# Intelligent-Driving-Laboratory/GOPS

Hardware: NVIDIA H100
Metric: batched env-steps/sec (FHADP rollout+update) (higher is better)
Workload: dtype f32

## Files before the change

### gops_b200/csrc/rollout_tc2.cuh

```cuda
#pragma once
#include "models.cuh"
#include "mlp_tc_full.cuh"
#include "tc2_probe.cuh"

namespace gops {
namespace tc2 {

constexpr int WGS = 3;
constexpr int GT = 64;
constexpr int NT2 = 128 * WGS;
constexpr int HPL = tcf::HPLANE, XPL = tcf::XPLANE;
constexpr int P_BYTES = 3 * HPL, Q_BYTES = 2 * HPL, XP_BYTES = 3 * XPL;
constexpr int GROUP_BYTES = P_BYTES + Q_BYTES + 2 * XP_BYTES;
constexpr int HDR_BYTES = 256;

__host__ __device__ inline size_t smem_bytes(int w_floats) {
  return HDR_BYTES + (size_t)w_floats * 4 + tcf::ONES_B + (size_t)WGS * GROUP_BYTES;
}

__device__ __forceinline__ void split2(f32x2::u64 X, uint32_t& p0, uint32_t& p1) {
  float r0, r1;
  f32x2::upk(X, r0, r1);
  asm("cvt.rn.bf16x2.f32 %0, %1, %2;" : "=r"(p0) : "f"(r1), "f"(r0));
  f32x2::upk(f32x2::fma(tcf::bf16x2_as_f32x2(p0), f32x2::rep(-1.f), X), r0, r1);
  asm("cvt.rn.bf16x2.f32 %0, %1, %2;" : "=r"(p1) : "f"(r1), "f"(r0));
}

__device__ __forceinline__ void red_add(float* p, float v) {
  asm volatile("red.global.add.f32 [%0], %1;" ::"l"(p), "f"(v) : "memory");
}
__device__ __forceinline__ void red_add2(float* p, float v0, float v1) {
  asm volatile("red.global.add.v2.f32 [%0], {%1, %2};" ::"l"(p), "f"(v0), "f"(v1) : "memory");
}

struct Grp {
  unsigned char* P;
  const float* Wsm;
  int g, t, c;
  int row;
  bool own;
  __device__ __forceinline__ unsigned char* Q() const { return P + P_BYTES; }
  __device__ __forceinline__ unsigned char* X(int k) const { return P + P_BYTES + Q_BYTES + (k & 1) * XP_BYTES; }
  __device__ __forceinline__ const unsigned char* ones() const {
    return reinterpret_cast<const unsigned char*>(Wsm) - tcf::ONES_B;
  }
  __device__ __forceinline__ const unsigned char* W1(const NetL& L) const { return reinterpret_cast<const unsigned char*>(Wsm + L.o_w1); }
  __device__ __forceinline__ const unsigned char* W2(const NetL& L) const { return reinterpret_cast<const unsigned char*>(Wsm + L.o_w2); }
  __device__ __forceinline__ const float* W3(const NetL& L) const { return Wsm + L.o_w3; }
  __device__ __forceinline__ const float* b1(const NetL& L) const { return Wsm + L.o_b1; }
  __device__ __forceinline__ const float* b2(const NetL& L) const { return Wsm + L.o_b2; }
  __device__ __forceinline__ const float* b3(const NetL& L) const { return Wsm + L.o_b3; }
};

__device__ __forceinline__ void publish(const Grp& G) {
  fence_proxy_async();
  wg::wg_sync(G.g);
}

template <int N, int TB, int KS>
__device__ __forceinline__ void mma6(float* d, const tcf::Op& A, const tcf::Op& B) {
  using namespace tcf;
  const uint64_t a0 = dsc(A, 0), a1 = dsc(A, 1), a2 = dsc(A, 2), b0 = dsc(B, 0), b1 = dsc(B, 1), b2 = dsc(B, 2);
  const uint64_t ka = A.kadv >> 4, kb = B.kadv >> 4;
#pragma unroll
  for (int ks = 0; ks < KS; ++ks) wg::mma_bf16<N, 0, TB>(d, a2 + ks * ka, b0 + ks * kb, ks > 0 ? 1u : 0u);
#pragma unroll
  for (int ks = 0; ks < KS; ++ks) wg::mma_bf16<N, 0, TB>(d, a0 + ks * ka, b2 + ks * kb, 1u);
#pragma unroll
  for (int ks = 0; ks < KS; ++ks) wg::mma_bf16<N, 0, TB>(d, a1 + ks * ka, b1 + ks * kb, 1u);
#pragma unroll
  for (int ks = 0; ks < KS; ++ks) wg::mma_bf16<N, 0, TB>(d, a1 + ks * ka, b0 + ks * kb, 1u);
#pragma unroll
  for (int ks = 0; ks < KS; ++ks) wg::mma_bf16<N, 0, TB>(d, a0 + ks * ka, b1 + ks * kb, 1u);
#pragma unroll
  for (int ks = 0; ks < KS; ++ks) wg::mma_bf16<N, 0, TB>(d, a0 + ks * ka, b0 + ks * kb, 1u);
}
template <int N, int KS>
__device__ __forceinline__ void mma_dw(float* d, const tcf::Op& A, const tcf::Op& B) {
  using namespace tcf;
  const uint64_t a0 = dsc(A, 0), a1 = dsc(A, 1), b0 = dsc(B, 0), b1 = dsc(B, 1);
  const uint64_t ka = A.kadv >> 4, kb = B.kadv >> 4;
#pragma unroll
  for (int ks = 0; ks < KS; ++ks) wg::mma_bf16<N, 0, 1>(d, a1 + ks * ka, b0 + ks * kb, ks > 0 ? 1u : 0u);
#pragma unroll
  for (int ks = 0; ks < KS; ++ks) wg::mma_bf16<N, 0, 1>(d, a0 + ks * ka, b1 + ks * kb, 1u);
#pragma unroll
  for (int ks = 0; ks < KS; ++ks) wg::mma_bf16<N, 0, 1>(d, a0 + ks * ka, b0 + ks * kb, 1u);
}
template <int N, int BP>
__device__ __forceinline__ void mma_wgrad(float* d, const tcf::Op& A, const tcf::Op& B) {
  using namespace tcf;
  const uint64_t ka = A.kadv >> 4, kb = B.kadv >> 4;
  uint32_t acc = 0u;
#pragma unroll
  for (int p = BP - 1; p >= 0; --p)
#pragma unroll
    for (int q = 1; q >= 0; --q) {
      const uint64_t a = dsc(A, q), b = dsc(B, p);
#pragma unroll
      for (int ks = 0; ks < GT / 16; ++ks) { wg::mma_bf16<N, 1, 1>(d, a + ks * ka, b + ks * kb, acc); acc = 1u; }
    }
}
__device__ __forceinline__ tcf::Op ones_op(const Grp& G) { return tcf::Op{smem_u32(G.ones()), 0u, 128u, 256u, 0u}; }

template <int NP>
__device__ __forceinline__ void frag_to_planes(unsigned char* buf, const Grp& G, const float* v) {
#pragma unroll
  for (int i = 0; i < 32; i += 2) {
    const int off = (i >> 2) * (GT * 16) + wg::frag_row(G.t, i) * 16 + 4 * G.c;
    uint32_t w0, w1, w2;
    if constexpr (NP == 3) tcf::split3(v[i], v[i + 1], w0, w1, w2);
    else split2(f32x2::pk(v[i], v[i + 1]), w0, w1);
    *reinterpret_cast<uint32_t*>(buf + off) = w0;
    *reinterpret_cast<uint32_t*>(buf + HPL + off) = w1;
    if constexpr (NP == 3) *reinterpret_cast<uint32_t*>(buf + 2 * HPL + off) = w2;
  }
}
template <int N, bool PAIRS>
__device__ __forceinline__ void red_frag(float* __restrict__ dst, int ld, int ncols, const float* d, int t) {
#pragma unroll
  for (int i = 0; i < N / 2; i += 2) {
    const int row = wg::frag_row(t, i), col = wg::frag_col(t, i);
    if constexpr (PAIRS) {
      red_add2(dst + row * ld + col, d[i], d[i + 1]);
    } else {
      if (col < ncols) red_add(dst + row * ld + col, d[i]);
      if (col + 1 < ncols) red_add(dst + row * ld + col + 1, d[i + 1]);
    }
  }
}
__device__ __forceinline__ void red_bias(float* __restrict__ dst, const float* d, const Grp& G) {
  if (G.c == 0) {
    red_add(dst + wg::frag_row(G.t, 0), d[0]);
    red_add(dst + wg::frag_row(G.t, 2), d[2]);
  }
}

template <int NS>
__device__ __forceinline__ void put_x(const Grp& G, unsigned char* x, const NetL& L, const float* st, float vt) {
  using namespace tcf;
  if (!G.own) return;
  float v[16];
#pragma unroll
  for (int f = 0; f < 16; ++f) v[f] = (f < NS && f < L.obs) ? st[f < NS ? f : 0] : 0.f;
  if (L.time_input) {
#pragma unroll
    for (int f = 0; f < 16; ++f)
      if (f == L.in - 1) v[f] = vt;
  }
  const int nch = L.in <= 8 ? 1 : 2;
#pragma unroll
  for (int ch = 0; ch < 2; ++ch) {
    if (ch >= nch) break;
    uint32_t w[3][4];
#pragma unroll
    for (int i = 0; i < 4; ++i) split3(v[8 * ch + 2 * i], v[8 * ch + 2 * i + 1], w[0][i], w[1][i], w[2][i]);
#pragma unroll
    for (int p = 0; p < 3; ++p)
      *reinterpret_cast<uint4*>(x + p * XPL + (ch * GT + G.row) * 16) = make_uint4(w[p][0], w[p][1], w[p][2], w[p][3]);
  }
}

#define GOPS_TC2_ACT_SWITCH(AF, act, M)     \
  if constexpr ((AF) >= 0) { M(AF); }       \
  else { GOPS_ACT_SWITCH(act, M) }

__device__ __forceinline__ void layer1_issue(const Grp& G, const NetL& L, const unsigned char* x, float* d) {
  using namespace tcf;
  publish(G);
  wg::fence();
  mma6<64, 0, 1>(d, k_act(x, XPL), k_w(G.W1(L), W1PLANE));
  wg::commit();
}
template <bool FULL, int AF>
__device__ __forceinline__ void layer1_finish(const Grp& G, const NetL& L, float* d, float* a1p) {
  wg::wait<0>();
  wg::reg_fence<32>(d);
#define GOPS_TC2_A1(A)                                                                             \
  _Pragma("unroll") for (int i = 0; i < 32; i += 2) {                                              \
    const f32x2::u64 pre = f32x2::add(f32x2::pk(d[i], d[i + 1]), f32x2::ld(G.b1(L) + wg::frag_col(G.t, i))); \
    if constexpr (FULL) act_fwd_grad_pair_t<A>(pre, d[i], d[i + 1], a1p[i], a1p[i + 1]);           \
    else act_fwd_pair_t<A>(pre, d[i], d[i + 1]);                                                   \
  }
  GOPS_TC2_ACT_SWITCH(AF, L.hact, GOPS_TC2_A1)
#undef GOPS_TC2_A1
  frag_to_planes<3>(G.P, G, d);
}

__device__ __forceinline__ void layer2_product(const Grp& G, const NetL& L, float* d) {
  using namespace tcf;
  publish(G);
  wg::fence();
  mma6<64, 0, 4>(d, k_act(G.P, HPL), k_w(G.W2(L), W2PLANE));
  wg::commit();
  wg::wait<0>();
  wg::reg_fence<32>(d);
}
template <int NA>
__device__ __forceinline__ bool live(int a, const NetL& L) { return NA == 1 || a < L.out; }

template <int NA>
__device__ __forceinline__ void output_sum(const Grp& G, const NetL& L, f32x2::u64 (*S)[NA], float* z) {
#pragma unroll
  for (int a = 0; a < NA; ++a) {
    z[a] = 0.f;
    if (live<NA>(a, L)) {
      float s[2];
#pragma unroll
      for (int q = 0; q < 2; ++q) {
        float s0, s1;
        f32x2::upk(S[q][a], s0, s1);
        s[q] = s0 + s1;
        s[q] += __shfl_xor_sync(0xffffffffu, s[q], 1);
        s[q] += __shfl_xor_sync(0xffffffffu, s[q], 2);
      }
      z[a] = G.b3(L)[a] + (G.c == 0 ? s[0] : s[1]);
    }
  }
}
template <int NA>
__device__ __forceinline__ void output_layer(const Grp& G, const NetL& L, const float* h, float* z) {
  f32x2::u64 S[2][NA];
#pragma unroll
  for (int a = 0; a < NA; ++a) S[0][a] = S[1][a] = f32x2::rep(0.f);
#pragma unroll
  for (int i = 0; i < 32; i += 2) {
    const int col = wg::frag_col(G.t, i), q = (i >> 1) & 1;
#pragma unroll
    for (int a = 0; a < NA; ++a)
      if (live<NA>(a, L)) S[q][a] = f32x2::fma(f32x2::ld(G.W3(L) + a * 64 + col), f32x2::pk(h[i], h[i + 1]), S[q][a]);
  }
  output_sum<NA>(G, L, S, z);
}

template <int AF, int NA>
__device__ __forceinline__ void layer2_out(const Grp& G, const NetL& L, float* z) {
  float d[32];
  layer2_product(G, L, d);
#define GOPS_TC2_A2(A)                                \
  _Pragma("unroll") for (int i = 0; i < 32; i += 2)   \
      act_fwd_pair_t<A>(f32x2::add(f32x2::pk(d[i], d[i + 1]), f32x2::ld(G.b2(L) + wg::frag_col(G.t, i))), d[i], d[i + 1]);
  GOPS_TC2_ACT_SWITCH(AF, L.hact, GOPS_TC2_A2)
#undef GOPS_TC2_A2
  output_layer<NA>(G, L, d, z);
}

template <int NA>
struct Acc3 {
  float w[NA][2];
  float b[NA];
};

template <int A, bool WANT_DW, bool WANT_Z, int NA>
__device__ __forceinline__ void delta2_epilogue(const Grp& G, const NetL& L, float* d, const float (*zr)[NA],
                                                Acc3<NA>& acc3, f32x2::u64 (*S)[NA]) {
  const int q4 = (G.t & 31) >> 2;
#pragma unroll
  for (int j = 0; j < 8; ++j) {
    const int col = 8 * j + 2 * G.c;
    float h[2][2];
#pragma unroll
    for (int q = 0; q < 2; ++q) {
      const int i = 4 * j + 2 * q;
      float g0, g1;
      act_fwd_grad_pair_t<A>(f32x2::add(f32x2::pk(d[i], d[i + 1]), f32x2::ld(G.b2(L) + col)), h[q][0], h[q][1], g0, g1);
      f32x2::u64 gs = f32x2::rep(0.f);
#pragma unroll
      for (int a = 0; a < NA; ++a)
        if (live<NA>(a, L)) gs = f32x2::fma(f32x2::ld(G.W3(L) + a * 64 + col), f32x2::rep(zr[q][a]), gs);
      uint32_t w0, w1;
      split2(f32x2::mul(f32x2::pk(g0, g1), gs), w0, w1);
      const int off = j * (GT * 16) + wg::frag_row(G.t, i) * 16 + 4 * G.c;
      *reinterpret_cast<uint32_t*>(G.Q() + off) = w0;
      *reinterpret_cast<uint32_t*>(G.Q() + HPL + off) = w1;
      if constexpr (WANT_Z) {
#pragma unroll
        for (int a = 0; a < NA; ++a)
          if (live<NA>(a, L)) S[q][a] = f32x2::fma(f32x2::ld(G.W3(L) + a * 64 + col), f32x2::pk(h[q][0], h[q][1]), S[q][a]);
      }
    }
    if constexpr (WANT_DW) {
#pragma unroll
      for (int a = 0; a < NA; ++a)
        if (live<NA>(a, L)) {
#pragma unroll
          for (int e = 0; e < 2; ++e) {
            float v = fmaf(zr[1][a], h[1][e], zr[0][a] * h[0][e]);
            v += __shfl_xor_sync(0xffffffffu, v, 4);
            v += __shfl_xor_sync(0xffffffffu, v, 8);
            v += __shfl_xor_sync(0xffffffffu, v, 16);
            if (q4 == j) acc3.w[a][e] += v;
          }
        }
    }
  }
}

template <bool WANT_DW, bool WANT_Z, int AF, int NA>
__device__ __forceinline__ void layer2_back(const Grp& G, const NetL& L, const float* zbar, float* z, Acc3<NA>& acc3) {
  float d[32];
  layer2_product(G, L, d);
  const int qb = (G.t & 31) & ~3;
  float zr[2][NA];
#pragma unroll
  for (int a = 0; a < NA; ++a) {
    zr[0][a] = __shfl_sync(0xffffffffu, zbar[a], qb);
    zr[1][a] = __shfl_sync(0xffffffffu, zbar[a], qb + 1);
  }
  f32x2::u64 S[2][NA];
#pragma unroll
  for (int a = 0; a < NA; ++a) S[0][a] = S[1][a] = f32x2::rep(0.f);
#define GOPS_TC2_A3(A) delta2_epilogue<A, WANT_DW, WANT_Z, NA>(G, L, d, zr, acc3, S);
  GOPS_TC2_ACT_SWITCH(AF, L.hact, GOPS_TC2_A3)
#undef GOPS_TC2_A3
  if constexpr (WANT_Z) output_sum<NA>(G, L, S, z);
  if constexpr (WANT_DW) {
#pragma unroll
    for (int a = 0; a < NA; ++a)
      if (live<NA>(a, L) && G.own) acc3.b[a] += zbar[a];
  }
}

template <bool WANT_DW, int NS, bool OVERLAP>
__device__ __forceinline__ void backprop(const Grp& G, const NetL& L, bool want_dx, float* __restrict__ part,
                                         const unsigned char* x, const float* a1p, float* dx, Probe& pr) {
  using namespace tcf;
  publish(G);
  constexpr bool overlap = WANT_DW && OVERLAP;
  float g1[32], w[32], wb[8];
  wg::fence();
  mma_dw<64, 4>(g1, k_act(G.Q(), HPL), mn_w(G.W2(L), W2PLANE));
  wg::commit();
  if constexpr (overlap) {
    mma_wgrad<64, 2>(w, mn_act(G.Q(), HPL), mn_act(G.P, HPL));
    mma_wgrad<16, 1>(wb, mn_act(G.Q(), HPL), ones_op(G));
    wg::commit();
    wg::wait<1>();
  } else {
    wg::wait<0>();
  }
  wg::reg_fence<32>(g1);
  if (!WANT_DW && !want_dx) return;
#pragma unroll
  for (int i = 0; i < 32; ++i) g1[i] *= a1p[i];
  if constexpr (WANT_DW) {
    if constexpr (!overlap) {
      wg::fence();
      mma_wgrad<64, 2>(w, mn_act(G.Q(), HPL), mn_act(G.P, HPL));
      mma_wgrad<16, 1>(wb, mn_act(G.Q(), HPL), ones_op(G));
      wg::commit();
    }
    wg::wait<0>();
    wg::reg_fence<32>(w);
    wg::reg_fence<8>(wb);
    red_frag<64, true>(part + L.g_w2, 64, 64, w, G.t);
    red_bias(part + L.g_b2, wb, G);
  }
  pr.stamp(kRevD2);
  wg::wg_sync(G.g);
  frag_to_planes<2>(G.Q(), G, g1);
  publish(G);
  float d[8], w1[8], wb1[8];
  if (want_dx) {
    wg::fence();
    mma_dw<16, 4>(d, k_act(G.Q(), HPL), mn_w(G.W1(L), W1PLANE));
    wg::commit();
  }
  if constexpr (WANT_DW) {
    wg::fence();
    mma_wgrad<16, 2>(w1, mn_act(G.Q(), HPL), mn_act(x, XPL));
    mma_wgrad<16, 1>(wb1, mn_act(G.Q(), HPL), ones_op(G));
    wg::commit();
  }
  wg::wait<0>();
  if constexpr (WANT_DW) {
    wg::reg_fence<8>(w1);
    wg::reg_fence<8>(wb1);
    red_frag<16, false>(part + L.g_w1, L.in, L.in, w1, G.t);
    red_bias(part + L.g_b1, wb1, G);
  }
  if (want_dx) {
    wg::reg_fence<8>(d);
    const int qb = (G.t & 31) & ~3;
#pragma unroll
    for (int j = 0; j < 2; ++j)
#pragma unroll
      for (int cc = 0; cc < 4; ++cc)
#pragma unroll
        for (int e = 0; e < 2; ++e) {
          const int f = 8 * j + 2 * cc + e;
          if (f < NS) {
            const float v0 = __shfl_sync(0xffffffffu, d[4 * j + e], qb + cc);
            const float v1 = __shfl_sync(0xffffffffu, d[4 * j + 2 + e], qb + cc);
            dx[f] = G.c == 0 ? v0 : v1;
          }
        }
  }
}

}

template <class M, int ALG, int AF, int NA, class W>
__global__ void __launch_bounds__(tc2::NT2, 1) rollout_tc2_kernel(const __grid_constant__ KParams p) {
  using namespace tc2;
  static_assert(M::KIND == 0, "wgmma rollout kernel: state == obs models");
  static_assert(NA == 1 || NA == MAXA, "wgmma rollout kernel: NA is MAXA or 1");
  constexpr int NS = M::NS, alg = ALG;
  extern __shared__ __align__(16) float smem[];
  unsigned char* sm = reinterpret_cast<unsigned char*>(smem);
  uint64_t* bars = reinterpret_cast<uint64_t*>(sm);
  unsigned char* ones = sm + HDR_BYTES;
  float* Wsm = reinterpret_cast<float*>(ones + tcf::ONES_B);
  unsigned char* gbase = reinterpret_cast<unsigned char*>(Wsm + p.w_floats);

  const int tid = threadIdx.x;
  const int warp = __shfl_sync(0xffffffffu, tid >> 5, 0);
  Grp G;
  G.g = warp >> 2;
  G.t = tid & 127;
  G.c = tid & 3;
  G.row = wg::frag_row(G.t, 2 * (G.c & 1));
  G.own = G.c < 2;
  G.P = gbase + G.g * GROUP_BYTES;
  G.Wsm = Wsm;
  const bool own = G.own;

  if (tid == 0) {
    mbar_init(bars, 1);
    fence_mbar_init();
  }
  if (tid < 256) {
    uint16_t* o16 = reinterpret_cast<uint16_t*>(ones);
    o16[tid] = (tid < 128 && (tid & 7) == 0) ? (uint16_t)0x3f80 : (uint16_t)0;
  }
  uint32_t wphase = 0;
  auto stage = [&](const float* gsrc, int floats) {
    __syncthreads();
    if (tid == 0) {
      fence_proxy_async();
      const uint32_t bytes = (uint32_t)floats * 4u;
      mbar_expect_tx(bars, bytes);
      for (uint32_t off = 0; off < bytes; off += 32768u) {
        const uint32_t n = bytes - off < 32768u ? bytes - off : 32768u;
        tma_bulk_g2s(reinterpret_cast<char*>(Wsm) + off, reinterpret_cast<const char*>(gsrc) + off, n, bars);
      }
    }
    mbar_wait(bars, wphase);
    wphase ^= 1u;
  };

  const NetL& P = p.pol;
  const NetL& V = p.val;
  const int H = p.horizon, obs_dim = P.obs, TCH = p.tape_ch;
  const int pout = NA == 1 ? 1 : P.out;
  const long long B = p.batch;
  const int slot = blockIdx.x * WGS + G.g, slots = gridDim.x * WGS;
  float* part = p.partial + (size_t)slot * p.part_stride;
  for (int i = G.t; i < p.part_stride; i += 128) part[i] = 0.f;
  float* tape = p.tape + (size_t)slot * (size_t)H * TCH * GT;
  Acc3<NA> acc3;
#pragma unroll
  for (int a = 0; a < NA; ++a) acc3.w[a][0] = acc3.w[a][1] = acc3.b[a] = 0.f;
  float loss_acc = 0.f, vmean_acc = 0.f, done_acc = 0.f;
  Probe pr;
  pr.init(G.t);

  for (int i = G.t; i < 2 * XP_BYTES / 16; i += 128) reinterpret_cast<uint4*>(G.X(0))[i] = make_uint4(0u, 0u, 0u, 0u);
  stage(p.blob_pol, P.blob);

  const long long nsub = (B + GT - 1) / GT;
  const long long s0 = nsub * slot / slots, s1 = nsub * (slot + 1) / slots;
  long long iters = s1 - s0;
  if (WGS > 1 && (alg == ALG_PIM || alg == ALG_PEV)) {
    for (int o = 0; o < WGS; ++o) {
      const long long os = (long long)blockIdx.x * WGS + o;
      const long long n = nsub * (os + 1) / slots - nsub * os / slots;
      iters = n > iters ? n : iters;
    }
  }

  for (long long it = 0; it < iters; ++it) {
    const long long sub = s0 + it;
    const bool have = sub < s1;
    const long long gs = sub * GT + G.row;
    const bool valid = own && have && gs < B;
    float st[NS];
#pragma unroll
    for (int f = 0; f < NS; ++f) st[f] = (valid && f < obs_dim) ? p.obs[gs * obs_dim + f] : 0.f;
    bool dn = valid ? (p.done[gs] != 0.f) : true;
    float vacc = 0.f;

    if (have) {
      for (int k = 0; k < H; ++k) {
        pr.mark();
        if (own) {
          if (alg == ALG_FHADP || alg == ALG_PIM) {
#pragma unroll
            for (int f = 0; f < NS; ++f) tape[(k * TCH + f) * GT + G.row] = st[f];
            tape[(k * TCH + NS) * GT + G.row] = dn ? 1.f : 0.f;
          }
        }
        float z[NA], d1[32];
        put_x<NS>(G, G.X(k), P, st, (float)(k + 1));
        layer1_issue(G, P, G.X(k), d1);
        layer1_finish<false, AF>(G, P, d1, nullptr);
        pr.stamp(kFwdL1);
        layer2_out<AF, NA>(G, P, z);
        pr.stamp(kFwdL2);
        if (own) {
          float a[NA], g[NA], apol[NA];
          if (alg == ALG_FHADP || alg == ALG_PIM) {
#pragma unroll
            for (int j = 0; j < NA; ++j)
              if (j < pout) tape[(k * TCH + NS + 1 + j) * GT + G.row] = z[j];
          }
          process_action<NA, W>(p, pout, z, a, g, apol);
          const bool active = valid && (p.mask_at_done ? !dn : true);
          float r = 0.f;
          if (valid) {
            wrapped_step<M, W>(p, obs_dim, st, a, active, r, dn);
            r = shape_reward(p, r);
            vacc += r * p.gpow[k];
          }
          if (alg == ALG_TRACE && valid) {
            const size_t row = (size_t)k * B + gs;
            if (p.tr_obs)
              for (int f = 0; f < obs_dim; ++f) p.tr_obs[row * obs_dim + f] = st[f];
            if (p.tr_act)
              for (int j = 0; j < pout; ++j) p.tr_act[row * pout + j] = apol[j];
            if (p.tr_rew) p.tr_rew[row] = r;
            if (p.tr_done) p.tr_done[row] = dn ? 1.f : 0.f;
          }
        }
        pr.stamp(kFwdDyn);
        pr.step(true);
      }
      if (valid && dn) done_acc += 1.f;
    }
    if (alg == ALG_TRACE) continue;

    float lam[NS];
#pragma unroll
    for (int f = 0; f < NS; ++f) lam[f] = 0.f;
    if (alg != ALG_FHADP) {
      stage(p.blob_vtg, V.blob);
      if (have) {
        const float gn = p.gpow[H];
        const bool term = valid && !dn;
        float zv[NA], zb[NA], d1[32], a1p[32];
#pragma unroll
        for (int j = 0; j < NA; ++j) zb[j] = zv[j] = 0.f;
        put_x<NS>(G, G.X(0), V, st, 0.f);
        layer1_issue(G, V, G.X(0), d1);
        if (alg == ALG_PIM) {
          float dx[NS];
          zb[0] = term ? -gn * p.inv_B : 0.f;
          layer1_finish<true, AF>(G, V, d1, a1p);
          layer2_back<false, true, AF, NA>(G, V, zb, zv, acc3);
          backprop<false, NS, NA == 1>(G, V, true, part, G.X(0), a1p, dx, pr);
          if (term) {
#pragma unroll
            for (int f = 0; f < NS; ++f)
              if (f < obs_dim) lam[f] = dx[f];
          }
        } else {
          layer1_finish<false, AF>(G, V, d1, nullptr);
          layer2_out<AF, NA>(G, V, zv);
        }
        if (term) vacc += gn * zv[0];
      }
    }

    if (alg == ALG_PEV) {
      stage(p.blob_val, V.blob);
      if (have) {
        float o0[NS];
#pragma unroll
        for (int f = 0; f < NS; ++f) o0[f] = (valid && f < obs_dim) ? p.obs[gs * obs_dim + f] : 0.f;
        float zv[NA], zb[NA], d1[32], a1p[32];
#pragma unroll
        for (int j = 0; j < NA; ++j) zb[j] = zv[j] = 0.f;
        put_x<NS>(G, G.X(0), V, o0, 0.f);
        layer1_issue(G, V, G.X(0), d1);
        layer1_finish<true, AF>(G, V, d1, a1p);
        layer2_out<AF, NA>(G, V, zv);
        if (valid) {
          const float diff = zv[0] - vacc;
          loss_acc += diff * diff * p.inv_B;
          vmean_acc += zv[0] * p.inv_B;
          zb[0] = 2.f * diff * p.inv_B;
        }
        layer2_back<true, false, AF, NA>(G, V, zb, nullptr, acc3);
        backprop<true, NS, NA == 1>(G, V, false, part, G.X(0), a1p, nullptr, pr);
      }
      stage(p.blob_pol, P.blob);
      continue;
    }

    if (valid) loss_acc += -vacc * p.inv_B;
    if (alg == ALG_PIM) {
      stage(p.blob_pol, P.blob);
    }
    if (!have) continue;

    float nst[NS];
    bool ndn = false;
    if (own) {
#pragma unroll
      for (int f = 0; f < NS; ++f) nst[f] = tape[((H - 1) * TCH + f) * GT + G.row];
      ndn = tape[((H - 1) * TCH + NS) * GT + G.row] != 0.f;
    }
    for (int k = H - 1; k >= 0; --k) {
      pr.mark();
      float zt[NA];
      const bool dnk = ndn;
#pragma unroll
      for (int f = 0; f < NS; ++f) st[f] = nst[f];
#pragma unroll
      for (int j = 0; j < NA; ++j) zt[j] = 0.f;
      if (own) {
#pragma unroll
        for (int j = 0; j < NA; ++j)
          if (j < pout) zt[j] = tape[(k * TCH + NS + 1 + j) * GT + G.row];
      }
      float d1[32], a1p[32];
      put_x<NS>(G, G.X(k), P, st, (float)(k + 1));
      layer1_issue(G, P, G.X(k), d1);
      pr.stamp(kRevL1);
      float zb[NA];
#pragma unroll
      for (int j = 0; j < NA; ++j) zb[j] = 0.f;
      const bool active = valid && (p.mask_at_done ? !dnk : true);
      if (own) {
        if (k > 0) {
#pragma unroll
          for (int f = 0; f < NS; ++f) nst[f] = tape[((k - 1) * TCH + f) * GT + G.row];
          ndn = tape[((k - 1) * TCH + NS) * GT + G.row] != 0.f;
        }
        if (active) {
          float a[NA], g[NA], abar[NA];
          process_action<NA, W>(p, pout, zt, a, g, nullptr);
#pragma unroll
          for (int j = 0; j < NA; ++j) abar[j] = 0.f;
          wrapped_step_bwd<M, NA, W>(p, obs_dim, st, a, reward_adjoint(p, k), lam, abar);
#pragma unroll
          for (int j = 0; j < NA; ++j) zb[j] = abar[j] * g[j];
        }
      }
      pr.stamp(kRevAdj);
      layer1_finish<true, AF>(G, P, d1, a1p);
      pr.stamp(kRevL1);
      layer2_back<true, false, AF, NA>(G, P, zb, nullptr, acc3);
      pr.stamp(kRevL2);
      float dx[NS];
      backprop<true, NS, NA == 1>(G, P, k > 0, part, G.X(k), a1p, dx, pr);
      if (active && k > 0) {
#pragma unroll
        for (int f = 0; f < NS; ++f)
          if (f < obs_dim) lam[f] += dx[f];
      }
      pr.stamp(kRevD1);
      pr.step(false);
    }
    wg::wg_sync(G.g);
  }

  wg::wg_sync(G.g);
  const int lane = G.t & 31, w4 = G.t >> 5;
  if (alg != ALG_TRACE) {
    const NetL& U = (alg == ALG_PEV) ? V : P;
    constexpr int stride = NA * 64 + NA;
    float* rg = reinterpret_cast<float*>(G.P);
#pragma unroll
    for (int a = 0; a < NA; ++a)
      if (live<NA>(a, U)) {
        const int col = 8 * (lane >> 2) + 2 * G.c;
        rg[w4 * stride + a * 64 + col] = acc3.w[a][0];
        rg[w4 * stride + a * 64 + col + 1] = acc3.w[a][1];
        float sb = acc3.b[a];
#pragma unroll
        for (int o = 16; o > 0; o >>= 1) sb += __shfl_xor_sync(0xffffffffu, sb, o);
        if (lane == 0) rg[w4 * stride + NA * 64 + a] = sb;
      }
    wg::wg_sync(G.g);
    for (int i = G.t; i < U.out * 64; i += 128) {
      const int a = i >> 6, j = i & 63;
      part[U.g_w3 + i] = (rg[a * 64 + j] + rg[stride + a * 64 + j]) + (rg[2 * stride + a * 64 + j] + rg[3 * stride + a * 64 + j]);
    }
    if (G.t < U.out)
      part[U.g_b3 + G.t] = (rg[NA * 64 + G.t] + rg[stride + NA * 64 + G.t]) +
                           (rg[2 * stride + NA * 64 + G.t] + rg[3 * stride + NA * 64 + G.t]);
    wg::wg_sync(G.g);
  }
  {
    float* sc = reinterpret_cast<float*>(G.P);
    if (own) { sc[G.row] = loss_acc; sc[GT + G.row] = vmean_acc; sc[2 * GT + G.row] = done_acc; }
    wg::wg_sync(G.g);
    if (G.t < 3) {
      const int nparam = (alg == ALG_PEV) ? V.nparam : P.nparam;
      float s = 0.f;
      for (int i = 0; i < GT; ++i) s += sc[G.t * GT + i];
      part[nparam + G.t] = s;
    }
  }
  pr.finish(alg, WGS);
}

}
```

### gops_b200/csrc/wgmma.cuh

```cuda
#pragma once
#include "common.cuh"

namespace gops {
namespace wg {

__device__ __forceinline__ uint64_t smem_desc(uint32_t saddr, uint32_t lbo_bytes, uint32_t sbo_bytes) {
  return (uint64_t)((saddr >> 4) & 0x3fffu) | ((uint64_t)((lbo_bytes >> 4) & 0x3fffu) << 16) |
         ((uint64_t)((sbo_bytes >> 4) & 0x3fffu) << 32);
}

__device__ __forceinline__ void fence() { asm volatile("wgmma.fence.sync.aligned;" ::: "memory"); }
__device__ __forceinline__ void commit() { asm volatile("wgmma.commit_group.sync.aligned;" ::: "memory"); }
template <int PENDING>
__device__ __forceinline__ void wait() { asm volatile("wgmma.wait_group.sync.aligned %0;" ::"n"(PENDING) : "memory"); }
template <int N>
__device__ __forceinline__ void reg_fence(float* d) {
#pragma unroll
  for (int i = 0; i < N; ++i) asm volatile("" : "+f"(d[i])::"memory");
}

template <int TA, int TB>
__device__ __forceinline__ void mma_bf16_n16(float* d, uint64_t a, uint64_t b, uint32_t acc) {
  asm volatile(
      "{\n.reg .pred p;\nsetp.ne.b32 p, %10, 0;\n"
      "wgmma.mma_async.sync.aligned.m64n16k16.f32.bf16.bf16 {%0, %1, %2, %3, %4, %5, %6, %7}, %8, %9, p, 1, 1, %11, %12;\n}\n"
      : "+f"(d[0]), "+f"(d[1]), "+f"(d[2]), "+f"(d[3]), "+f"(d[4]), "+f"(d[5]), "+f"(d[6]), "+f"(d[7])
      : "l"(a), "l"(b), "r"(acc), "n"(TA), "n"(TB)
      : "memory");
}

template <int TA, int TB>
__device__ __forceinline__ void mma_bf16_n32(float* d, uint64_t a, uint64_t b, uint32_t acc) {
  asm volatile(
      "{\n.reg .pred p;\nsetp.ne.b32 p, %18, 0;\n"
      "wgmma.mma_async.sync.aligned.m64n32k16.f32.bf16.bf16 {%0, %1, %2, %3, %4, %5, %6, %7, %8, %9, %10, %11, %12, %13, %14, %15}, %16, %17, p, 1, 1, %19, %20;\n}\n"
      : "+f"(d[0]), "+f"(d[1]), "+f"(d[2]), "+f"(d[3]), "+f"(d[4]), "+f"(d[5]), "+f"(d[6]), "+f"(d[7]), "+f"(d[8]), "+f"(d[9]), "+f"(d[10]), "+f"(d[11]), "+f"(d[12]), "+f"(d[13]), "+f"(d[14]), "+f"(d[15])
      : "l"(a), "l"(b), "r"(acc), "n"(TA), "n"(TB)
      : "memory");
}

template <int TA, int TB>
__device__ __forceinline__ void mma_bf16_n64(float* d, uint64_t a, uint64_t b, uint32_t acc) {
  asm volatile(
      "{\n.reg .pred p;\nsetp.ne.b32 p, %34, 0;\n"
      "wgmma.mma_async.sync.aligned.m64n64k16.f32.bf16.bf16 {%0, %1, %2, %3, %4, %5, %6, %7, %8, %9, %10, %11, %12, %13, %14, %15, %16, %17, %18, %19, %20, %21, %22, %23, %24, %25, %26, %27, %28, %29, %30, %31}, %32, %33, p, 1, 1, %35, %36;\n}\n"
      : "+f"(d[0]), "+f"(d[1]), "+f"(d[2]), "+f"(d[3]), "+f"(d[4]), "+f"(d[5]), "+f"(d[6]), "+f"(d[7]), "+f"(d[8]), "+f"(d[9]), "+f"(d[10]), "+f"(d[11]), "+f"(d[12]), "+f"(d[13]), "+f"(d[14]), "+f"(d[15]), "+f"(d[16]), "+f"(d[17]), "+f"(d[18]), "+f"(d[19]), "+f"(d[20]), "+f"(d[21]), "+f"(d[22]), "+f"(d[23]), "+f"(d[24]), "+f"(d[25]), "+f"(d[26]), "+f"(d[27]), "+f"(d[28]), "+f"(d[29]), "+f"(d[30]), "+f"(d[31])
      : "l"(a), "l"(b), "r"(acc), "n"(TA), "n"(TB)
      : "memory");
}

template <int TA, int TB>
__device__ __forceinline__ void mma_bf16_n128(float* d, uint64_t a, uint64_t b, uint32_t acc) {
  asm volatile(
      "{\n.reg .pred p;\nsetp.ne.b32 p, %66, 0;\n"
      "wgmma.mma_async.sync.aligned.m64n128k16.f32.bf16.bf16 {%0, %1, %2, %3, %4, %5, %6, %7, %8, %9, %10, %11, %12, %13, %14, %15, %16, %17, %18, %19, %20, %21, %22, %23, %24, %25, %26, %27, %28, %29, %30, %31, %32, %33, %34, %35, %36, %37, %38, %39, %40, %41, %42, %43, %44, %45, %46, %47, %48, %49, %50, %51, %52, %53, %54, %55, %56, %57, %58, %59, %60, %61, %62, %63}, %64, %65, p, 1, 1, %67, %68;\n}\n"
      : "+f"(d[0]), "+f"(d[1]), "+f"(d[2]), "+f"(d[3]), "+f"(d[4]), "+f"(d[5]), "+f"(d[6]), "+f"(d[7]), "+f"(d[8]), "+f"(d[9]), "+f"(d[10]), "+f"(d[11]), "+f"(d[12]), "+f"(d[13]), "+f"(d[14]), "+f"(d[15]), "+f"(d[16]), "+f"(d[17]), "+f"(d[18]), "+f"(d[19]), "+f"(d[20]), "+f"(d[21]), "+f"(d[22]), "+f"(d[23]), "+f"(d[24]), "+f"(d[25]), "+f"(d[26]), "+f"(d[27]), "+f"(d[28]), "+f"(d[29]), "+f"(d[30]), "+f"(d[31]), "+f"(d[32]), "+f"(d[33]), "+f"(d[34]), "+f"(d[35]), "+f"(d[36]), "+f"(d[37]), "+f"(d[38]), "+f"(d[39]), "+f"(d[40]), "+f"(d[41]), "+f"(d[42]), "+f"(d[43]), "+f"(d[44]), "+f"(d[45]), "+f"(d[46]), "+f"(d[47]), "+f"(d[48]), "+f"(d[49]), "+f"(d[50]), "+f"(d[51]), "+f"(d[52]), "+f"(d[53]), "+f"(d[54]), "+f"(d[55]), "+f"(d[56]), "+f"(d[57]), "+f"(d[58]), "+f"(d[59]), "+f"(d[60]), "+f"(d[61]), "+f"(d[62]), "+f"(d[63])
      : "l"(a), "l"(b), "r"(acc), "n"(TA), "n"(TB)
      : "memory");
}

__device__ __forceinline__ void mma_tf32_n64(float* d, uint64_t a, uint64_t b, uint32_t acc) {
  asm volatile(
      "{\n.reg .pred p;\nsetp.ne.b32 p, %34, 0;\n"
      "wgmma.mma_async.sync.aligned.m64n64k8.f32.tf32.tf32 {%0, %1, %2, %3, %4, %5, %6, %7, %8, %9, %10, %11, %12, %13, %14, %15, %16, %17, %18, %19, %20, %21, %22, %23, %24, %25, %26, %27, %28, %29, %30, %31}, %32, %33, p, 1, 1;\n}\n"
      : "+f"(d[0]), "+f"(d[1]), "+f"(d[2]), "+f"(d[3]), "+f"(d[4]), "+f"(d[5]), "+f"(d[6]), "+f"(d[7]), "+f"(d[8]), "+f"(d[9]), "+f"(d[10]), "+f"(d[11]), "+f"(d[12]), "+f"(d[13]), "+f"(d[14]), "+f"(d[15]), "+f"(d[16]), "+f"(d[17]), "+f"(d[18]), "+f"(d[19]), "+f"(d[20]), "+f"(d[21]), "+f"(d[22]), "+f"(d[23]), "+f"(d[24]), "+f"(d[25]), "+f"(d[26]), "+f"(d[27]), "+f"(d[28]), "+f"(d[29]), "+f"(d[30]), "+f"(d[31])
      : "l"(a), "l"(b), "r"(acc)
      : "memory");
}

template <int N, int TA, int TB>
__device__ __forceinline__ void mma_bf16(float* d, uint64_t a, uint64_t b, uint32_t acc) {
  static_assert(N == 16 || N == 32 || N == 64 || N == 128, "wgmma bf16 tile width");
  if constexpr (N == 16) mma_bf16_n16<TA, TB>(d, a, b, acc);
  else if constexpr (N == 32) mma_bf16_n32<TA, TB>(d, a, b, acc);
  else if constexpr (N == 64) mma_bf16_n64<TA, TB>(d, a, b, acc);
  else mma_bf16_n128<TA, TB>(d, a, b, acc);
}

__device__ __forceinline__ int frag_row(int t, int i) { return 16 * (t >> 5) + ((t & 31) >> 2) + 8 * ((i >> 1) & 1); }
__device__ __forceinline__ int frag_col(int t, int i) { return 8 * (i >> 2) + 2 * (t & 3) + (i & 1); }

__device__ __forceinline__ void split(float x, float& hi, float& lo) {
  hi = __uint_as_float((__float_as_uint(x) + 0x1000u) & 0xffffe000u);
  lo = x - hi;
}

__device__ __forceinline__ void wg_sync(int g) { asm volatile("bar.sync %0, 128;" ::"r"(1 + g) : "memory"); }

}
}
```

Baseline: 1.296 billion.

## Feed layer-2 A operand from registers and accumulate W2 grads in shared memory

Forward layer-2 wgmma now takes its bf16-split hidden activations directly from registers instead of writing them to shared-memory planes, which skips the frag_to_planes store and the barrier when the full tape is not needed. The W2 weight gradient is accumulated per group in a shared-memory fp32 buffer across steps and written to global memory once at the end, replacing per-step vector red.global atomics. The double-buffered X input is collapsed to a single buffer with an explicit group sync in put_x, which frees shared memory for the accumulator but serialises reuse of X.

```diff
diff --git a/gops_b200/csrc/rollout_tc2.cuh b/gops_b200/csrc/rollout_tc2.cuh
--- a/gops_b200/csrc/rollout_tc2.cuh
+++ b/gops_b200/csrc/rollout_tc2.cuh
@@ -11,7 +11,8 @@
 constexpr int NT2 = 128 * WGS;
 constexpr int HPL = tcf::HPLANE, XPL = tcf::XPLANE;
 constexpr int P_BYTES = 3 * HPL, Q_BYTES = 2 * HPL, XP_BYTES = 3 * XPL;
-constexpr int GROUP_BYTES = P_BYTES + Q_BYTES + 2 * XP_BYTES;
+constexpr int ACC_BYTES = 64 * 64 * 4;
+constexpr int GROUP_BYTES = P_BYTES + Q_BYTES + XP_BYTES + ACC_BYTES;
 constexpr int HDR_BYTES = 256;
 
 __host__ __device__ inline size_t smem_bytes(int w_floats) {
@@ -29,8 +30,10 @@
 __device__ __forceinline__ void red_add(float* p, float v) {
   asm volatile("red.global.add.f32 [%0], %1;" ::"l"(p), "f"(v) : "memory");
 }
-__device__ __forceinline__ void red_add2(float* p, float v0, float v1) {
-  asm volatile("red.global.add.v2.f32 [%0], {%1, %2};" ::"l"(p), "f"(v0), "f"(v1) : "memory");
+__device__ __forceinline__ float add_ftz(float a, float b) {
+  float r;
+  asm("add.rn.ftz.f32 %0, %1, %2;" : "=f"(r) : "f"(a), "f"(b));
+  return r;
 }
 
 struct Grp {
@@ -40,7 +43,8 @@
   int row;
   bool own;
   __device__ __forceinline__ unsigned char* Q() const { return P + P_BYTES; }
-  __device__ __forceinline__ unsigned char* X(int k) const { return P + P_BYTES + Q_BYTES + (k & 1) * XP_BYTES; }
+  __device__ __forceinline__ unsigned char* X() const { return P + P_BYTES + Q_BYTES; }
+  __device__ __forceinline__ float* acc() const { return reinterpret_cast<float*>(P + P_BYTES + Q_BYTES + XP_BYTES); }
   __device__ __forceinline__ const unsigned char* ones() const {
     return reinterpret_cast<const unsigned char*>(Wsm) - tcf::ONES_B;
   }
@@ -74,6 +78,24 @@
   for (int ks = 0; ks < KS; ++ks) wg::mma_bf16<N, 0, TB>(d, a0 + ks * ka, b1 + ks * kb, 1u);
 #pragma unroll
   for (int ks = 0; ks < KS; ++ks) wg::mma_bf16<N, 0, TB>(d, a0 + ks * ka, b0 + ks * kb, 1u);
+}
+template <int KS>
+__device__ __forceinline__ void mma6_ra(float* d, const uint32_t (*a)[4 * KS], const tcf::Op& B) {
+  using namespace tcf;
+  const uint64_t b0 = dsc(B, 0), b1 = dsc(B, 1), b2 = dsc(B, 2);
+  const uint64_t kb = B.kadv >> 4;
+#pragma unroll
+  for (int ks = 0; ks < KS; ++ks) wg::mma_bf16_n64_ra<0>(d, a[2] + 4 * ks, b0 + ks * kb, ks > 0 ? 1u : 0u);
+#pragma unroll
+  for (int ks = 0; ks < KS; ++ks) wg::mma_bf16_n64_ra<0>(d, a[0] + 4 * ks, b2 + ks * kb, 1u);
+#pragma unroll
+  for (int ks = 0; ks < KS; ++ks) wg::mma_bf16_n64_ra<0>(d, a[1] + 4 * ks, b1 + ks * kb, 1u);
+#pragma unroll
+  for (int ks = 0; ks < KS; ++ks) wg::mma_bf16_n64_ra<0>(d, a[1] + 4 * ks, b0 + ks * kb, 1u);
+#pragma unroll
+  for (int ks = 0; ks < KS; ++ks) wg::mma_bf16_n64_ra<0>(d, a[0] + 4 * ks, b1 + ks * kb, 1u);
+#pragma unroll
+  for (int ks = 0; ks < KS; ++ks) wg::mma_bf16_n64_ra<0>(d, a[0] + 4 * ks, b0 + ks * kb, 1u);
 }
 template <int N, int KS>
 __device__ __forceinline__ void mma_dw(float* d, const tcf::Op& A, const tcf::Op& B) {
@@ -116,30 +138,38 @@
     if constexpr (NP == 3) *reinterpret_cast<uint32_t*>(buf + 2 * HPL + off) = w2;
   }
 }
-template <int N, bool PAIRS>
+template <int N>
 __device__ __forceinline__ void red_frag(float* __restrict__ dst, int ld, int ncols, const float* d, int t) {
 #pragma unroll
   for (int i = 0; i < N / 2; i += 2) {
     const int row = wg::frag_row(t, i), col = wg::frag_col(t, i);
-    if constexpr (PAIRS) {
-      red_add2(dst + row * ld + col, d[i], d[i + 1]);
-    } else {
-      if (col < ncols) red_add(dst + row * ld + col, d[i]);
-      if (col + 1 < ncols) red_add(dst + row * ld + col + 1, d[i + 1]);
-    }
-  }
-}
-__device__ __forceinline__ void red_bias(float* __restrict__ dst, const float* d, const Grp& G) {
+    if (col < ncols) red_add(dst + row * ld + col, d[i]);
+    if (col + 1 < ncols) red_add(dst + row * ld + col + 1, d[i + 1]);
+  }
+}
+__device__ __forceinline__ void acc_frag(const Grp& G, const float* d) {
+#pragma unroll
+  for (int i = 0; i < 32; i += 2) {
+    float2* s = reinterpret_cast<float2*>(G.acc()) + (i >> 1) * 128 + G.t;
+    float2 v = *s;
+    v.x = add_ftz(v.x, d[i]);
+    v.y = add_ftz(v.y, d[i + 1]);
+    *s = v;
+  }
+}
+__device__ __forceinline__ void red_bias(const Grp& G, float* part, int off, const float* d) {
   if (G.c == 0) {
-    red_add(dst + wg::frag_row(G.t, 0), d[0]);
-    red_add(dst + wg::frag_row(G.t, 2), d[2]);
+    red_add(part + off + wg::frag_row(G.t, 0), d[0]);
+    red_add(part + off + wg::frag_row(G.t, 2), d[2]);
   }
 }
 
 template <int NS>
-__device__ __forceinline__ void put_x(const Grp& G, unsigned char* x, const NetL& L, const float* st, float vt) {
-  using namespace tcf;
+__device__ __forceinline__ void put_x(const Grp& G, const NetL& L, const float* st, float vt) {
+  using namespace tcf;
+  wg::wg_sync(G.g);
   if (!G.own) return;
+  unsigned char* x = G.X();
   float v[16];
 #pragma unroll
   for (int f = 0; f < 16; ++f) v[f] = (f < NS && f < L.obs) ? st[f < NS ? f : 0] : 0.f;
@@ -165,11 +195,11 @@
   if constexpr ((AF) >= 0) { M(AF); }       \
   else { GOPS_ACT_SWITCH(act, M) }
 
-__device__ __forceinline__ void layer1_issue(const Grp& G, const NetL& L, const unsigned char* x, float* d) {
+__device__ __forceinline__ void layer1_issue(const Grp& G, const NetL& L, float* d) {
   using namespace tcf;
   publish(G);
   wg::fence();
-  mma6<64, 0, 1>(d, k_act(x, XPL), k_w(G.W1(L), W1PLANE));
+  mma6<64, 0, 1>(d, k_act(G.X(), XPL), k_w(G.W1(L), W1PLANE));
   wg::commit();
 }
 template <bool FULL, int AF>
@@ -184,7 +214,7 @@
   }
   GOPS_TC2_ACT_SWITCH(AF, L.hact, GOPS_TC2_A1)
 #undef GOPS_TC2_A1
-  frag_to_planes<3>(G.P, G, d);
+  if constexpr (FULL) frag_to_planes<3>(G.P, G, d);
 }
 
 __device__ __forceinline__ void layer2_product(const Grp& G, const NetL& L, float* d) {
@@ -196,6 +226,19 @@
   wg::wait<0>();
   wg::reg_fence<32>(d);
 }
+__device__ __forceinline__ void layer2_product_ra(const Grp& G, const NetL& L, const float* h, float* d) {
+  using namespace tcf;
+  uint32_t a[3][16];
+#pragma unroll
+  for (int i = 0; i < 32; i += 2) split3(h[i], h[i + 1], a[0][i >> 1], a[1][i >> 1], a[2][i >> 1]);
+  wg::fence();
+  mma6_ra<4>(d, a, k_w(G.W2(L), W2PLANE));
+  wg::commit();
+  wg::wait<0>();
+  wg::reg_fence<32>(d);
+#pragma unroll
+  for (int p = 0; p < 3; ++p) wg::reg_fence_u32<16>(a[p]);
+}
 template <int NA>
 __device__ __forceinline__ bool live(int a, const NetL& L) { return NA == 1 || a < L.out; }
 
@@ -233,10 +276,11 @@
   output_sum<NA>(G, L, S, z);
 }
 
-template <int AF, int NA>
-__device__ __forceinline__ void layer2_out(const Grp& G, const NetL& L, float* z) {
+template <int AF, int NA, bool REGA>
+__device__ __forceinline__ void layer2_out(const Grp& G, const NetL& L, const float* h, float* z) {
   float d[32];
-  layer2_product(G, L, d);
+  if constexpr (REGA) layer2_product_ra(G, L, h, d);
+  else layer2_product(G, L, d);
 #define GOPS_TC2_A2(A)                                \
   _Pragma("unroll") for (int i = 0; i < 32; i += 2)   \
       act_fwd_pair_t<A>(f32x2::add(f32x2::pk(d[i], d[i + 1]), f32x2::ld(G.b2(L) + wg::frag_col(G.t, i))), d[i], d[i + 1]);
@@ -323,7 +367,7 @@
 
 template <bool WANT_DW, int NS, bool OVERLAP>
 __device__ __forceinline__ void backprop(const Grp& G, const NetL& L, bool want_dx, float* __restrict__ part,
-                                         const unsigned char* x, const float* a1p, float* dx, Probe& pr) {
+                                         const float* a1p, float* dx, Probe& pr) {
   using namespace tcf;
   publish(G);
   constexpr bool overlap = WANT_DW && OVERLAP;
@@ -353,8 +397,8 @@
     wg::wait<0>();
     wg::reg_fence<32>(w);
     wg::reg_fence<8>(wb);
-    red_frag<64, true>(part + L.g_w2, 64, 64, w, G.t);
-    red_bias(part + L.g_b2, wb, G);
+    acc_frag(G, w);
+    red_bias(G, part, L.g_b2, wb);
   }
   pr.stamp(kRevD2);
   wg::wg_sync(G.g);
@@ -368,7 +412,7 @@
   }
   if constexpr (WANT_DW) {
     wg::fence();
-    mma_wgrad<16, 2>(w1, mn_act(G.Q(), HPL), mn_act(x, XPL));
+    mma_wgrad<16, 2>(w1, mn_act(G.Q(), HPL), mn_act(G.X(), XPL));
     mma_wgrad<16, 1>(wb1, mn_act(G.Q(), HPL), ones_op(G));
     wg::commit();
   }
@@ -376,8 +420,8 @@
   if constexpr (WANT_DW) {
     wg::reg_fence<8>(w1);
     wg::reg_fence<8>(wb1);
-    red_frag<16, false>(part + L.g_w1, L.in, L.in, w1, G.t);
-    red_bias(part + L.g_b1, wb1, G);
+    red_frag<16>(part + L.g_w1, L.in, L.in, w1, G.t);
+    red_bias(G, part, L.g_b1, wb1);
   }
   if (want_dx) {
     wg::reg_fence<8>(d);
@@ -465,7 +509,7 @@
   Probe pr;
   pr.init(G.t);
 
-  for (int i = G.t; i < 2 * XP_BYTES / 16; i += 128) reinterpret_cast<uint4*>(G.X(0))[i] = make_uint4(0u, 0u, 0u, 0u);
+  for (int i = G.t; i < (XP_BYTES + ACC_BYTES) / 16; i += 128) reinterpret_cast<uint4*>(G.X())[i] = make_uint4(0u, 0u, 0u, 0u);
   stage(p.blob_pol, P.blob);
 
   const long long nsub = (B + GT - 1) / GT;
@@ -501,11 +545,11 @@
           }
         }
         float z[NA], d1[32];
-        put_x<NS>(G, G.X(k), P, st, (float)(k + 1));
-        layer1_issue(G, P, G.X(k), d1);
+        put_x<NS>(G, P, st, (float)(k + 1));
+        layer1_issue(G, P, d1);
         layer1_finish<false, AF>(G, P, d1, nullptr);
         pr.stamp(kFwdL1);
-        layer2_out<AF, NA>(G, P, z);
+        layer2_out<AF, NA, true>(G, P, d1, z);
         pr.stamp(kFwdL2);
         if (own) {
           float a[NA], g[NA], apol[NA];
@@ -550,14 +594,14 @@
         float zv[NA], zb[NA], d1[32], a1p[32];
 #pragma unroll
         for (int j = 0; j < NA; ++j) zb[j] = zv[j] = 0.f;
-        put_x<NS>(G, G.X(0), V, st, 0.f);
-        layer1_issue(G, V, G.X(0), d1);
+        put_x<NS>(G, V, st, 0.f);
+        layer1_issue(G, V, d1);
         if (alg == ALG_PIM) {
           float dx[NS];
           zb[0] = term ? -gn * p.inv_B : 0.f;
           layer1_finish<true, AF>(G, V, d1, a1p);
           layer2_back<false, true, AF, NA>(G, V, zb, zv, acc3);
-          backprop<false, NS, NA == 1>(G, V, true, part, G.X(0), a1p, dx, pr);
+          backprop<false, NS, NA == 1>(G, V, true, part, a1p, dx, pr);
           if (term) {
 #pragma unroll
             for (int f = 0; f < NS; ++f)
@@ -565,7 +609,7 @@
           }
         } else {
           layer1_finish<false, AF>(G, V, d1, nullptr);
-          layer2_out<AF, NA>(G, V, zv);
+          layer2_out<AF, NA, true>(G, V, d1, zv);
         }
         if (term) vacc += gn * zv[0];
       }
@@ -580,10 +624,10 @@
         float zv[NA], zb[NA], d1[32], a1p[32];
 #pragma unroll
         for (int j = 0; j < NA; ++j) zb[j] = zv[j] = 0.f;
-        put_x<NS>(G, G.X(0), V, o0, 0.f);
-        layer1_issue(G, V, G.X(0), d1);
+        put_x<NS>(G, V, o0, 0.f);
+        layer1_issue(G, V, d1);
         layer1_finish<true, AF>(G, V, d1, a1p);
-        layer2_out<AF, NA>(G, V, zv);
+        layer2_out<AF, NA, false>(G, V, d1, zv);
         if (valid) {
           const float diff = zv[0] - vacc;
           loss_acc += diff * diff * p.inv_B;
@@ -591,7 +635,7 @@
           zb[0] = 2.f * diff * p.inv_B;
         }
         layer2_back<true, false, AF, NA>(G, V, zb, nullptr, acc3);
-        backprop<true, NS, NA == 1>(G, V, false, part, G.X(0), a1p, nullptr, pr);
+        backprop<true, NS, NA == 1>(G, V, false, part, a1p, nullptr, pr);
       }
       stage(p.blob_pol, P.blob);
       continue;
@@ -624,8 +668,8 @@
           if (j < pout) zt[j] = tape[(k * TCH + NS + 1 + j) * GT + G.row];
       }
       float d1[32], a1p[32];
-      put_x<NS>(G, G.X(k), P, st, (float)(k + 1));
-      layer1_issue(G, P, G.X(k), d1);
+      put_x<NS>(G, P, st, (float)(k + 1));
+      layer1_issue(G, P, d1);
       pr.stamp(kRevL1);
       float zb[NA];
 #pragma unroll
@@ -653,7 +697,7 @@
       layer2_back<true, false, AF, NA>(G, P, zb, nullptr, acc3);
       pr.stamp(kRevL2);
       float dx[NS];
-      backprop<true, NS, NA == 1>(G, P, k > 0, part, G.X(k), a1p, dx, pr);
+      backprop<true, NS, NA == 1>(G, P, k > 0, part, a1p, dx, pr);
       if (active && k > 0) {
 #pragma unroll
         for (int f = 0; f < NS; ++f)
@@ -662,13 +706,16 @@
       pr.stamp(kRevD1);
       pr.step(false);
     }
-    wg::wg_sync(G.g);
   }
 
   wg::wg_sync(G.g);
   const int lane = G.t & 31, w4 = G.t >> 5;
   if (alg != ALG_TRACE) {
     const NetL& U = (alg == ALG_PEV) ? V : P;
+#pragma unroll
+    for (int i = 0; i < 32; i += 2)
+      *reinterpret_cast<float2*>(part + U.g_w2 + wg::frag_row(G.t, i) * 64 + wg::frag_col(G.t, i)) =
+          reinterpret_cast<const float2*>(G.acc())[(i >> 1) * 128 + G.t];
     constexpr int stride = NA * 64 + NA;
     float* rg = reinterpret_cast<float*>(G.P);
 #pragma unroll
diff --git a/gops_b200/csrc/wgmma.cuh b/gops_b200/csrc/wgmma.cuh
--- a/gops_b200/csrc/wgmma.cuh
+++ b/gops_b200/csrc/wgmma.cuh
@@ -59,6 +59,21 @@
       : "memory");
 }
 
+template <int TB>
+__device__ __forceinline__ void mma_bf16_n64_ra(float* d, const uint32_t* a, uint64_t b, uint32_t acc) {
+  asm volatile(
+      "{\n.reg .pred p;\nsetp.ne.b32 p, %37, 0;\n"
+      "wgmma.mma_async.sync.aligned.m64n64k16.f32.bf16.bf16 {%0, %1, %2, %3, %4, %5, %6, %7, %8, %9, %10, %11, %12, %13, %14, %15, %16, %17, %18, %19, %20, %21, %22, %23, %24, %25, %26, %27, %28, %29, %30, %31}, {%32, %33, %34, %35}, %36, p, 1, 1, %38;\n}\n"
+      : "+f"(d[0]), "+f"(d[1]), "+f"(d[2]), "+f"(d[3]), "+f"(d[4]), "+f"(d[5]), "+f"(d[6]), "+f"(d[7]), "+f"(d[8]), "+f"(d[9]), "+f"(d[10]), "+f"(d[11]), "+f"(d[12]), "+f"(d[13]), "+f"(d[14]), "+f"(d[15]), "+f"(d[16]), "+f"(d[17]), "+f"(d[18]), "+f"(d[19]), "+f"(d[20]), "+f"(d[21]), "+f"(d[22]), "+f"(d[23]), "+f"(d[24]), "+f"(d[25]), "+f"(d[26]), "+f"(d[27]), "+f"(d[28]), "+f"(d[29]), "+f"(d[30]), "+f"(d[31])
+      : "r"(a[0]), "r"(a[1]), "r"(a[2]), "r"(a[3]), "l"(b), "r"(acc), "n"(TB)
+      : "memory");
+}
+template <int N>
+__device__ __forceinline__ void reg_fence_u32(uint32_t* a) {
+#pragma unroll
+  for (int i = 0; i < N; ++i) asm volatile("" : "+r"(a[i])::"memory");
+}
+
 __device__ __forceinline__ void mma_tf32_n64(float* d, uint64_t a, uint64_t b, uint32_t acc) {
   asm volatile(
       "{\n.reg .pred p;\nsetp.ne.b32 p, %34, 0;\n"
```

Result: faster. 1.378 billion (median of 6 runs) (+6.3%).
